# gudovskiy/contextflow

Hardware: AMD Instinct MI355X
Metric: samples/s fwd+logdet (log p(x) (B,M)), CIFAR-10C conv flow (higher is better)
Workload: dtype f32

## Files before the change

contextflow_amd/csrc/cf_step.hip:

```cpp
#include "cf_step_common.h"
#include <cstdlib>

namespace {

constexpr int kPrepBatch = 16;
struct StepPackBatch {
    const float *Wm[kPrepBatch], *t[kPrepBatch], *logs[kPrepBatch], *w1[kPrepBatch], *b1[kPrepBatch], *w2[kPrepBatch], *b2[kPrepBatch],
        *w3[kPrepBatch], *b3[kPrepBatch];
    float* ws[kPrepBatch];
    int pieces;
    int w24;
};
template <class G>
__global__ __launch_bounds__(256) void k_step_pack(const StepPackBatch pb) {
    const int bi = blockIdx.y;
    const float* __restrict__ Wm = pb.Wm[bi]; const float* __restrict__ t = pb.t[bi]; const float* __restrict__ logs = pb.logs[bi];
    const float* __restrict__ w1 = pb.w1[bi]; const float* __restrict__ b1 = pb.b1[bi]; const float* __restrict__ w2 = pb.w2[bi];
    const float* __restrict__ b2 = pb.b2[bi]; const float* __restrict__ w3 = pb.w3[bi]; const float* __restrict__ b3 = pb.b3[bi];
    float* __restrict__ ws = pb.ws[bi];
    const int gtid = blockIdx.x * 256 + threadIdx.x, gsz = gridDim.x * 256;
    if (gtid == 0) {
        float s = 0.f;
        for (int c = 0; c < G::C; ++c) s += logs[c];
        ws[0] = (float)G::HW * ws[1] + s;
// ... 34 lines not shown
    }
    {
        constexpr int HID = G::HID;
        const double Gm[4][3] = {{1, 0, 0}, {.5, .5, .5}, {.5, -.5, .5}, {0, 0, 1}};
        for (int e = gtid; e < 16 * HID * HID; e += gsz) {
            const int jj = e & 3, ln = (e >> 2) & 63, q = e >> 8;
            const int kg = q % G::KG4, rt16 = (q / G::KG4) % G::RT16, pos = q / (G::KG4 * G::RT16);
            const int co = rt16 * 16 + (ln & 15), ci = 4 * (4 * kg + jj) + (ln >> 4), xi = pos >> 2, nu = pos & 3;
            const float* wk = w2 + ((int64_t)co * HID + ci) * 9;
            double u = 0.0;
            for (int a = 0; a < 3; ++a)
                for (int b = 0; b < 3; ++b) u += Gm[xi][a] * Gm[nu][b] * (double)wk[a * 3 + b];
            ws[G::OFF_AW + e] = (float)u;
        }
        if (G::KB32 > 0 && G::HID == 32 && pb.pieces) {
            unsigned short* wb = reinterpret_cast<unsigned short*>(ws + G::OFF_AWB);
            for (int e = gtid; e < 16 * G::RT16 * G::KB32 * 64 * 8; e += gsz) {
                const int j = e & 7, ln = (e >> 3) & 63, q = e >> 9;
                const int kb = q % G::KB32, rt16 = (q / G::KB32) % G::RT16, pos = q / (G::KB32 * G::RT16);
                const int co = rt16 * 16 + (ln & 15), ci = 32 * kb + 4 * j + (ln >> 4), xi = pos >> 2, nu = pos & 3;
                const float* wk = w2 + ((int64_t)co * HID + ci) * 9;
                double u = 0.0;
                for (int a = 0; a < 3; ++a)
                    for (int b = 0; b < 3; ++b) u += Gm[xi][a] * Gm[nu][b] * (double)wk[a * 3 + b];
                const float uf = (float)u;
                const unsigned u0 = __float_as_uint(uf) & 0xffff0000u;
                const float r1 = uf - __uint_as_float(u0);
                const unsigned u1 = __float_as_uint(r1) & 0xffff0000u;
                const float r2 = r1 - __uint_as_float(u1);
                const unsigned pc[3] = {u0, u1, __float_as_uint(r2)};
#pragma unroll
                for (int pz = 0; pz < 3; ++pz)
                    wb[((((int64_t)(pos * G::RT16 + rt16) * G::KB32 + kb) * 3 + pz) * 64 + ln) * 8 + j] = (unsigned short)(pc[pz] >> 16);
            }
        }
        if (G::KB32 > 0 && G::HID == 32 && pb.pieces) {
            unsigned short* wb = reinterpret_cast<unsigned short*>(ws + G::OFF_ADB);
            for (int e = gtid; e < 9 * G::RT16 * G::KB32 * 64 * 8; e += gsz) {
                const int j = e & 7, ln = (e >> 3) & 63, q = e >> 9;
                const int kb = q % G::KB32, rt16 = (q / G::KB32) % G::RT16, tap = q / (G::KB32 * G::RT16);
                const int co = rt16 * 16 + (ln & 15), ci = 32 * kb + 8 * (ln >> 4) + j;
                const float uf = w2[((int64_t)co * HID + ci) * 9 + tap];
                const unsigned u0 = __float_as_uint(uf) & 0xffff0000u;
                const float r1 = uf - __uint_as_float(u0);
                const unsigned u1 = __float_as_uint(r1) & 0xffff0000u;
                const float r2 = r1 - __uint_as_float(u1);
                const unsigned pc[3] = {u0, u1, __float_as_uint(r2)};
#pragma unroll
                for (int pz = 0; pz < 3; ++pz)
                    wb[((((int64_t)(tap * G::RT16 + rt16) * G::KB32 + kb) * 3 + pz) * 64 + ln) * 8 + j] = (unsigned short)(pc[pz] >> 16);
            }
        }
    }
    if (G::H == 4 && G::W == 4 && pb.w24) {
        constexpr int HID = G::HID;
        const double G2[4][3] = {{1, 0, 0}, {.5, .5, .5}, {.5, -.5, .5}, {0, 0, 1}};
        const double G4[6][3] = {{4, 0, 0}, {2. / 3, 2. / 3, 2. / 3}, {2. / 3, -2. / 3, 2. / 3}, {-8. / 3, -4. / 3, -2. / 3},
                                 {-8. / 3, 4. / 3, -2. / 3}, {0, 0, 1}};
        for (int e = gtid; e < 24 * HID * HID; e += gsz) {
            const int jj = e & 3, ln = (e >> 2) & 63, q = e >> 8;
            const int kg = q % G::KG4, rt16 = (q / G::KG4) % G::RT16, pos = q / (G::KG4 * G::RT16);
            const int co = rt16 * 16 + (ln & 15), ci = 4 * (4 * kg + jj) + (ln >> 4), xi = pos / 6, nu = pos % 6;
            const float* wk = w2 + ((int64_t)co * HID + ci) * 9;
            double u = 0.0;
            for (int a = 0; a < 3; ++a)
                for (int b = 0; b < 3; ++b) u += G2[xi][a] * G4[nu][b] * (double)wk[a * 3 + b];
            ws[G::OFF_AW24 + e] = (float)u;
        }
    }
    if constexpr (G::RS16) {
        constexpr int C = G::C, HID = G::HID, HALF = G::HALF;
        for (int p = gtid; p < C; p += gsz) { ws[G::OFF_RB0 + p] = -t[p] * expf(-logs[p]); ws[G::OFF_RB3 + p] = b3[p]; }
        for (int p = gtid; p < HID; p += gsz) { ws[G::OFF_RB1 + p] = b1[p]; ws[G::OFF_RB2 + p] = b2[p]; }
        auto split16 = [](int e, int NG, int& rt, int& gi, int& row, int& kk, int& j) {
            j = e & 3; const int ln = (e >> 2) & 63, q = e >> 8; gi = q % NG; rt = q / NG; row = 16 * rt + (ln & 15); kk = ln >> 4;
        };
        int rt, gi, row, kk, j;
        for (int e = gtid; e < (C / 16) * (C / 16) * 256; e += gsz) {
            split16(e, C / 16, rt, gi, row, kk, j);
            const int k = 4 * (4 * gi + j) + kk;
            ws[G::OFF_RA0 + e] = expf(-logs[row]) * Wm[row * C + k];
        }
        for (int e = gtid; e < (HID / 16) * (HALF / 16) * 256; e += gsz) {
            split16(e, HALF / 16, rt, gi, row, kk, j);
            ws[G::OFF_RA1 + e] = w1[row * HALF + 4 * (4 * gi + j) + kk];
        }
        for (int e = gtid; e < (HID / 16) * 9 * (HID / 16) * 256; e += gsz) {
            split16(e, 9 * (HID / 16), rt, gi, row, kk, j);
            const int tap = gi / (HID / 16), ci = 4 * (4 * (gi % (HID / 16)) + j) + kk;
            ws[G::OFF_RA2 + e] = w2[(row * HID + ci) * 9 + tap];
        }
        for (int e = gtid; e < (C / 16) * (HID / 16) * 256; e += gsz) {
            split16(e, HID / 16, rt, gi, row, kk, j);
            ws[G::OFF_RA3 + e] = w3[row * HID + 4 * (4 * gi + j) + kk];
        }
    }
    if constexpr (G::SMALL) {
        for (int p = gtid; p < 16; p += gsz) {
            const int ch = chan_of_row16<G>(p);
            ws[G::OFF_SB0 + p] = ch >= 0 ? -t[ch] * expf(-logs[ch]) : 0.f;
            ws[G::OFF_SB3 + p] = ch >= 0 ? b3[ch] : 0.f;
        }
        for (int e = gtid; e < G::SG0 * 256; e += gsz) {
            const int jj = e & 3, ln = (e >> 2) & 63, gg = e >> 8, ch = chan_of_row16<G>(ln & 15), k = 4 * (4 * gg + jj) + (ln >> 4);
            ws[G::OFF_SA0 + e] = (ch >= 0 && k < G::C) ? expf(-logs[ch]) * Wm[ch * G::C + k] : 0.f;
        }
        for (int e = gtid; e < G::SG3 * 256; e += gsz) {
// ... 992 lines not shown
    float* Xp = H1 + C * PIX;
#pragma unroll
    for (int rt = 0; rt < I::RTI; ++rt)
#pragma unroll
        for (int q = 0; q < PTW; ++q)
#pragma unroll
            for (int r = 0; r < 16; ++r) {
                const int row = rt * 32 + tile_row(r, lk);
                if (row < C) Xp[row * PIX + pix[q]] = acc[rt][q][r];
            }
    cf_wave_sync();
    if (x_unsq) rows_store_unsq<G>(x, Xp, b0, B, wave, lane);
    else rows_store<G, C>(x, Xp, b0, 0, B, wave, lane);
}

template <class G>
int launch_prepare_inv(const float* Wm, const float* t, const float* logs, float* wsi, hipStream_t s) {
    using I = GeoInv<G>;
    int rc = cf_slogdet_inverse(Wm, G::C, wsi + I::WS_FLOATS, wsi + I::OFF_WINV, (cf_stream_t)s);
    if (rc) return rc;
    k_step_pack_inv<G><<<dim3(16), dim3(256), 0, s>>>(t, logs, wsi);
    return 0;
}

static int g_bf16_split = -1;
static int bf16_split_mode() {
    static const int v = [] { const char* e = getenv("CONTEXTFLOW_BF16_SPLIT"); return (e && (e[0] == '1' || e[0] == '2')) ? e[0] - '0' : 0; }();
    return g_bf16_split < 0 ? v : g_bf16_split;
}
static bool bf16_split_enabled() { return bf16_split_mode() != 0; }

template <class G>
int launch_step_inv(const float* z, float* x, const float* ws, const float* wsi, int B, int64_t zbs, int x_unsq, hipStream_t s) {
    constexpr size_t lds_bytes = (size_t)G::LDS_FLOATS * sizeof(float);
    if (lds_bytes > 64 * 1024) {
        static std::atomic<uint64_t> raised{0};
        if (int rc_ = cf_raise_dynamic_lds((const void*)k_flow_step_inv<G>, 160 * 1024, raised, __func__)) return rc_;
    }
    k_flow_step_inv<G><<<dim3((B + G::SPW - 1) / G::SPW), dim3(256), lds_bytes, s>>>(z, x, ws, wsi, B, zbs, x_unsq);
    return 0;
}


}

static bool direct_conv_only() {
    static const bool v = [] { const char* e = getenv("CONTEXTFLOW_DIRECT_CONV"); return e && e[0] == '1'; }();
    return v;
}
static bool wino24_enabled() {
    static const bool v = [] { const char* e = getenv("CONTEXTFLOW_WINO24"); return !(e && e[0] == '0'); }();
    return v;
}

extern "C" {

int cf_flow_step_supported(int C, int H, int W, int kh, int kw) {
    return (kh == 3 && kw == 3 && shape_id(C, H, W) >= 0) ? 1 : 0;
}

int64_t cf_flow_step_ws_bytes(int C, int H, int W) {
    switch (shape_id(C, H, W)) {
        case 0: return (int64_t)G8::WS_FLOATS * 4;
        case 1: return (int64_t)G16::WS_FLOATS * 4;
        case 2: return (int64_t)G32::WS_FLOATS * 4;
        case 3: return (int64_t)G64::WS_FLOATS * 4;
    }
    return 0;
}

int cf_flow_step_prepare_batch(int n, const float* const* Wm, const float* const* t, const float* const* logs, const float* const* w1,
                               const float* const* b1, const float* const* w2, const float* const* b2, const float* const* w3,
                               const float* const* b3, void* const* ws, float* const* winv, int C, int H, int W, cf_stream_t stream) {
    CF_REQUIRE(n >= 0 && Wm && t && logs && w1 && b1 && w2 && b2 && w3 && b3 && ws);
    const int sid = shape_id(C, H, W);
    if (sid < 0) { cf_set_error("cf_flow_step_prepare: shape (%d,%d,%d) unsupported", C, H, W); return CF_ERR_UNSUPPORTED; }
    for (int i0 = 0; i0 < n; i0 += kPrepBatch) {
        const int m = n - i0 < kPrepBatch ? n - i0 : kPrepBatch;
        StepPackBatch pb{};
        pb.pieces = bf16_split_enabled() ? 1 : 0;
        pb.w24 = (wino24_enabled() && !direct_conv_only()) ? 1 : 0;
        for (int i = 0; i < m; ++i) {
            const int j = i0 + i;
            CF_REQUIRE(Wm[j] && t[j] && logs[j] && w1[j] && b1[j] && w2[j] && b2[j] && w3[j] && b3[j] && ws[j] &&
                       (reinterpret_cast<uintptr_t>(ws[j]) & 15) == 0 && (!winv || winv[j]));
            pb.Wm[i] = Wm[j]; pb.t[i] = t[j]; pb.logs[i] = logs[j]; pb.w1[i] = w1[j]; pb.b1[i] = b1[j]; pb.w2[i] = w2[j]; pb.b2[i] = b2[j];
            pb.w3[i] = w3[j]; pb.b3[i] = b3[j]; pb.ws[i] = (float*)ws[j];
        }
        int rc = 0;
        switch (sid) {
            case 0: rc = launch_prepare<G8>(pb, m, winv ? winv + i0 : nullptr, cf_s(stream)); break;
            case 1: rc = launch_prepare<G16>(pb, m, winv ? winv + i0 : nullptr, cf_s(stream)); break;
            case 2: rc = launch_prepare<G32>(pb, m, winv ? winv + i0 : nullptr, cf_s(stream)); break;
            default: rc = launch_prepare<G64>(pb, m, winv ? winv + i0 : nullptr, cf_s(stream)); break;
        }
        if (rc) return rc;
        CF_LAUNCH_CHECK();
    }
    return 0;
}

int cf_flow_step_prepare(const float* Wm, const float* t, const float* logs, const float* w1, const float* b1,
                         const float* w2, const float* b2, const float* w3, const float* b3, void* ws, int C, int H, int W,
                         cf_stream_t stream) {
    CF_REQUIRE(Wm && t && logs && w1 && b1 && w2 && b2 && w3 && b3 && ws && (reinterpret_cast<uintptr_t>(ws) & 15) == 0);
    return cf_flow_step_prepare_batch(1, &Wm, &t, &logs, &w1, &b1, &w2, &b2, &w3, &b3, &ws, nullptr, C, H, W, stream);
// ... 71 lines not shown
    if (dbg != nullptr && variant == 3 && shape_id(C, H, W) <= 1 && shape_id(C, H, W) >= 0) {
        if (shape_id(C, H, W) == 0)
            rc = in_squeeze ? launch_step_small<G8s, true, true>(x, z, ldj_acc, w, B, x_bstride, cf_s(stream), dbg)
                            : launch_step_small<G8s, false, true>(x, z, ldj_acc, w, B, x_bstride, cf_s(stream), dbg);
        else
            rc = in_squeeze ? launch_step_small<G16s, true, true>(x, z, ldj_acc, w, B, x_bstride, cf_s(stream), dbg)
                            : launch_step_small<G16s, false, true>(x, z, ldj_acc, w, B, x_bstride, cf_s(stream), dbg);
        if (rc) return rc;
        CF_LAUNCH_CHECK();
        return 0;
    }
    if (dbg != nullptr) {
        CF_REQUIRE(variant == 0);
#define CF_STEPD(G) rc = in_squeeze ? launch_step<G, true, 0, false, true>(x, z, ldj_acc, w, B, x_bstride, dbg, flags, cf_s(stream)) \
                                    : launch_step<G, false, 0, false, true>(x, z, ldj_acc, w, B, x_bstride, dbg, flags, cf_s(stream))
        switch (shape_id(C, H, W)) {
            case 0: CF_STEPD(G8); break;
            case 1: CF_STEPD(G16); break;
            case 2: CF_STEPD(G32); break;
            case 3: CF_STEPD(G64); break;
            default: cf_set_error("cf_flow_step_fwd_debug: shape (%d,%d,%d) unsupported", C, H, W); return CF_ERR_UNSUPPORTED;
        }
#undef CF_STEPD
        if (rc) return rc;
        CF_LAUNCH_CHECK();
        return 0;
    }
    switch (shape_id(C, H, W) * 8 + variant) {
        case 0: CF_STEP(G8); break;
        case 3: rc = in_squeeze ? launch_step_small<G8s, true>(x, z, ldj_acc, w, B, x_bstride, cf_s(stream))
                                : launch_step_small<G8s, false>(x, z, ldj_acc, w, B, x_bstride, cf_s(stream)); break;
        case 8: CF_STEP(G16); break;
        case 9: CF_STEP(G16v1); break;
        case 10: CF_STEP(G16v2); break;
        case 11: rc = in_squeeze ? launch_step_small<G16s, true>(x, z, ldj_acc, w, B, x_bstride, cf_s(stream))
                                : launch_step_small<G16s, false>(x, z, ldj_acc, w, B, x_bstride, cf_s(stream)); break;
        case 16: CF_STEP(G32); break;
        case 17: CF_STEP(G32v1); break;
        case 18: CF_STEP(G32v2); break;
        case 19: CF_STEP(G32v3); break;
        case 24: CF_STEP(G64); break;
        case 25: CF_STEP(G64v1); break;
        case 26: CF_STEP(G64v2); break;
        case 27: CF_STEP(G64v3); break;
        case 4: rc = in_squeeze ? launch_step_small<G8w, true>(x, z, ldj_acc, w, B, x_bstride, cf_s(stream))
                               : launch_step_small<G8w, false>(x, z, ldj_acc, w, B, x_bstride, cf_s(stream)); break;
        case 14: rc = in_squeeze ? launch_step_small<G16wb, true>(x, z, ldj_acc, w, B, x_bstride, cf_s(stream))
                                 : launch_step_small<G16wb, false>(x, z, ldj_acc, w, B, x_bstride, cf_s(stream)); break;
        case 15: rc = in_squeeze ? launch_step_small<G16db, true>(x, z, ldj_acc, w, B, x_bstride, cf_s(stream))
                                 : launch_step_small<G16db, false>(x, z, ldj_acc, w, B, x_bstride, cf_s(stream)); break;
        case 12: rc = in_squeeze ? launch_step_small<G16w, true>(x, z, ldj_acc, w, B, x_bstride, cf_s(stream))
                                : launch_step_small<G16w, false>(x, z, ldj_acc, w, B, x_bstride, cf_s(stream)); break;
        case 20: CF_STEP(G32w); break;
        case 28: CF_STEP(G64w); break;
        case 29: CF_STEP(G64w2); break;
        case 30: CF_STEP(G64w24); break;
        default: cf_set_error("cf_flow_step_fwd: shape (%d,%d,%d) variant %d unsupported", C, H, W, variant); return CF_ERR_UNSUPPORTED;
    }
#undef CF_STEP
    if (rc) return rc;
    CF_LAUNCH_CHECK();
    return 0;
}

int cf_flow_step_chain_max_batch(int C, int H, int W) {
    switch (shape_id(C, H, W)) {
        case 0: case 1: return direct_conv_only() ? 0 : 1024;
        case 2: return 512;
        case 3: return CF_RS16_MAXB < CF_RS_MAXB_C64 ? CF_RS16_MAXB : CF_RS_MAXB_C64;
    }
    return 0;
}

int cf_flow_step_fwd_chain(const float* x, float* z, float* ldj_acc, const void* const* ws, int n, int B, int C, int H, int W,
                           int64_t x_bstride, int in_squeeze, cf_stream_t stream) {
    if (B == 0 || n == 0) return 0;
    CF_REQUIRE(x && z && ldj_acc && ws && n >= 1 && n <= kChain && B > 0 && x_bstride >= (int64_t)C * H * W);
    CF_REQUIRE((reinterpret_cast<uintptr_t>(x) & 15) == 0 && (reinterpret_cast<uintptr_t>(z) & 15) == 0 && x_bstride % 4 == 0);
    const int sid = shape_id(C, H, W);
    if (sid < 0 || B > cf_flow_step_chain_max_batch(C, H, W)) {
        cf_set_error("cf_flow_step_fwd_chain: shape (%d,%d,%d) at a batch of %d is not a chained case", C, H, W, B);
        return CF_ERR_UNSUPPORTED;
    }
    WsChain wc{};
    for (int i = 0; i < n; ++i) { CF_REQUIRE(ws[i]); wc.ws[i] = (const float*)ws[i]; }
    hipStream_t s = cf_s(stream);
    switch (sid) {
        case 0: in_squeeze ? launch_step_small_chain<G8w, true>(x, z, ldj_acc, wc, n, B, x_bstride, s)
                           : launch_step_small_chain<G8w, false>(x, z, ldj_acc, wc, n, B, x_bstride, s); break;
        case 1: in_squeeze ? launch_step_small_chain<G16w, true>(x, z, ldj_acc, wc, n, B, x_bstride, s)
                           : launch_step_small_chain<G16w, false>(x, z, ldj_acc, wc, n, B, x_bstride, s); break;
        case 2: in_squeeze ? launch_step_rs_chain<G32, 2, true>(x, z, ldj_acc, wc, n, B, x_bstride, s)
                           : launch_step_rs_chain<G32, 2, false>(x, z, ldj_acc, wc, n, B, x_bstride, s); break;
        default:
            if (in_squeeze) k_flow_step_rs16_chain<G64, true><<<dim3(B), dim3(256), 0, s>>>(x, z, ldj_acc, wc, n, B, x_bstride);
            else k_flow_step_rs16_chain<G64, false><<<dim3(B), dim3(256), 0, s>>>(x, z, ldj_acc, wc, n, B, x_bstride);
    }
    CF_LAUNCH_CHECK();
    return 0;
}

int cf_bf16_split(int on) {
    if (on >= 0) g_bf16_split = on > 2 ? 1 : on;
    return bf16_split_mode();
}

int cf_flow_step_fwd(const float* x, float* z, float* ldj_acc, const void* ws, int B, int C, int H, int W,
                     int64_t x_bstride, int in_squeeze, cf_stream_t stream) {
    int flags = 0;
    const int sid = shape_id(C, H, W);
    if ((sid == 2 && B < 256 * G32::SPW) || (sid == 3 && B < 256 * G64::SPW)) flags = 2 << 16;
    if (sid == 0 || sid == 1) flags = 3 << 16;
    const bool direct_only = direct_conv_only();
    if (!direct_only && (sid == 0 || sid == 1 || (sid == 2 && B >= 256 * G32::SPW))) flags = 4 << 16;
    if (!direct_only && sid == 3 && B >= 256 * G64w2::SPW) flags = (wino24_enabled() ? 6 : 5) << 16;
    if (!direct_only && sid == 1 && bf16_split_mode() == 1) flags = 6 << 16;
    if (!direct_only && sid == 1 && bf16_split_mode() == 2 && B >= 1024) flags = 7 << 16;
    if ((sid == 2 && B <= 512) || (sid == 3 && B <= CF_RS_MAXB_C64)) {
        CF_REQUIRE(x && z && ldj_acc && ws && B >= 0 && x_bstride >= (int64_t)C * H * W);
        if (B == 0) return 0;
        const float* w = (const float*)ws;
        if (sid == 3 && B <= CF_RS16_MAXB) {
            if (in_squeeze) k_flow_step_rs16<G64, true><<<dim3(B), dim3(256), 0, cf_s(stream)>>>(x, z, ldj_acc, w, B, x_bstride, kNoTape);
            else k_flow_step_rs16<G64, false><<<dim3(B), dim3(256), 0, cf_s(stream)>>>(x, z, ldj_acc, w, B, x_bstride, kNoTape);
            CF_LAUNCH_CHECK();
            return 0;
        }
        if (sid == 2) { if (in_squeeze) launch_step_rs<G32, 2, true>(x, z, ldj_acc, w, B, x_bstride, cf_s(stream));
                        else launch_step_rs<G32, 2, false>(x, z, ldj_acc, w, B, x_bstride, cf_s(stream)); }
        else          { if (in_squeeze) launch_step_rs<G64, 1, true>(x, z, ldj_acc, w, B, x_bstride, cf_s(stream));
                        else launch_step_rs<G64, 1, false>(x, z, ldj_acc, w, B, x_bstride, cf_s(stream)); }
        CF_LAUNCH_CHECK();
        return 0;
    }
    return cf_flow_step_fwd_debug(x, z, ldj_acc, ws, B, C, H, W, x_bstride, in_squeeze, nullptr, flags, stream);
}

int64_t cf_flow_step_macs(int B, int C, int H, int W, int pass) {
    const int sid = shape_id(C, H, W);
    if (sid < 0 || pass < 0 || pass > 3) return 0;
    const int64_t direct = 40ll * C * C * H * W, wino = 20ll * C * C * H * W, wino24 = 16ll * C * C * H * W;
    if (pass == 2 || direct_conv_only()) return direct;
    if (pass == 3) return wino;
    if (sid == 3 && pass == 0 && wino24_enabled() && B >= 256 * G64w2::SPW) return wino24;
    bool w;
    if (sid == 0) w = pass == 0;
    else if (sid == 1) w = true;
    else if (sid == 2) w = B >= 256 * G32::SPW;
    else w = B >= 256 * G64w2::SPW;
    return w ? wino : direct;
}

int64_t cf_flow_step_tape_aux_bytes(int B, int C, int H, int W) {
    return shape_id(C, H, W) < 0 ? 0 : tape_aux_bytes(B, C, H, W);
}

int cf_flow_step_fwd_taped(const float* x, float* z, float* ldj_acc, const void* ws, float* t_y0, float* t_h1, float* t_h2,
                           void* t_aux, int B, int C, int H, int W, int64_t x_bstride, int in_squeeze, cf_stream_t stream) {
    if (B == 0) return 0;
    CF_REQUIRE(x && z && ldj_acc && ws && t_y0 && t_h1 && t_h2 && t_aux && x_bstride >= (int64_t)C * H * W && x_bstride % 4 == 0);
    CF_REQUIRE((reinterpret_cast<uintptr_t>(x) & 15) == 0 && (reinterpret_cast<uintptr_t>(z) & 15) == 0 &&
               (reinterpret_cast<uintptr_t>(t_y0) & 15) == 0 && (reinterpret_cast<uintptr_t>(t_h1) & 15) == 0 &&
               (reinterpret_cast<uintptr_t>(t_h2) & 15) == 0 && (reinterpret_cast<uintptr_t>(t_aux) & 15) == 0);
    const float* w = (const float*)ws;
    const StepTape tp = make_tape(t_y0, t_h1, t_h2, t_aux, B, C, H, W);
    const bool direct_only = direct_conv_only();
    int rc = 0;
#define CF_STEPT(G) rc = in_squeeze ? launch_step<G, true, 0, true>(x, z, ldj_acc, w, B, x_bstride, nullptr, 0, cf_s(stream), nullptr, tp) \
                                    : launch_step<G, false, 0, true>(x, z, ldj_acc, w, B, x_bstride, nullptr, 0, cf_s(stream), nullptr, tp)
    switch (shape_id(C, H, W)) {
        case 0: rc = in_squeeze ? launch_step_small<G8s, true, false, true>(x, z, ldj_acc, w, B, x_bstride, cf_s(stream), nullptr, tp)
                                : launch_step_small<G8s, false, false, true>(x, z, ldj_acc, w, B, x_bstride, cf_s(stream), nullptr, tp); break;
        case 1: if (direct_only) rc = in_squeeze ? launch_step_small<G16s, true, false, true>(x, z, ldj_acc, w, B, x_bstride, cf_s(stream), nullptr, tp)
                                                 : launch_step_small<G16s, false, false, true>(x, z, ldj_acc, w, B, x_bstride, cf_s(stream), nullptr, tp);
                else rc = in_squeeze ? launch_step_small<G16w, true, false, true>(x, z, ldj_acc, w, B, x_bstride, cf_s(stream), nullptr, tp)
                                     : launch_step_small<G16w, false, false, true>(x, z, ldj_acc, w, B, x_bstride, cf_s(stream), nullptr, tp);
                break;
        case 2: if (B <= 512) rc = in_squeeze ? launch_step_rs<G32, 2, true, true>(x, z, ldj_acc, w, B, x_bstride, cf_s(stream), tp)
                                              : launch_step_rs<G32, 2, false, true>(x, z, ldj_acc, w, B, x_bstride, cf_s(stream), tp);
                else if (B < 256 * G32::SPW) CF_STEPT(G32v2); else if (direct_only) CF_STEPT(G32); else CF_STEPT(G32w); break;
        case 3: if (B <= CF_RS16_MAXB) {
                    if (in_squeeze) k_flow_step_rs16<G64, true, true><<<dim3(B), dim3(256), 0, cf_s(stream)>>>(x, z, ldj_acc, w, B, x_bstride, tp);
                    else k_flow_step_rs16<G64, false, true><<<dim3(B), dim3(256), 0, cf_s(stream)>>>(x, z, ldj_acc, w, B, x_bstride, tp);
                }
                else if (!direct_only && B >= 256 * G64w2::SPW) CF_STEPT(G64w2); else if (B < 256 * G64::SPW) CF_STEPT(G64v2); else CF_STEPT(G64); break;
        default: cf_set_error("cf_flow_step_fwd_taped: shape (%d,%d,%d) unsupported", C, H, W); return CF_ERR_UNSUPPORTED;
    }
#undef CF_STEPT
    if (rc) return rc;
    CF_LAUNCH_CHECK();
    return 0;
}

int cf_flow_step_fwd_ctx(const float* x, float* z, float* ldj_acc, const void* ws, const float* sbias, int mode, int B, int C,
                         int H, int W, int64_t x_bstride, cf_stream_t stream) {
    if (B == 0) return 0;
    const bool keep_direct = (mode & 4) != 0;
// ... 51 lines not shown
```

contextflow_amd/csrc/cf_step_common.h:

```cpp
#pragma once
#include <type_traits>
#include "cf_common.h"
#include <math.h>

namespace {


typedef float f32x16 __attribute__((ext_vector_type(16)));

constexpr int kWaves = 4;

template <int C_, int H_, int W_, int SPW_, int PIPE_ = 1, int ABL_ = 0, int PATCH_ = 0>
struct Geo {
    static constexpr int C = C_, H = H_, W = W_, SPW = SPW_, PIPE = PIPE_, ABL = ABL_, PATCH = PATCH_;
    static constexpr int HW = H * W;
    static constexpr int PIX = SPW * HW;
    static constexpr int HALF = C / 2;
    static constexpr int HID = 2 * C;
    static constexpr int NPT = PIX / 32;
    static constexpr int PTW = NPT / kWaves;
    static constexpr int HP = HALF <= 16 ? 16 : 32;
    static constexpr int R03 = 2 * HP;
    static constexpr int RT03 = R03 / 32;
    static constexpr int RT1 = (HID + 31) / 32;
    static constexpr int R1 = RT1 * 32;
    static constexpr int KS0 = C / 2, KS1 = HALF / 2, KS3 = HID / 2;
    static constexpr int NG0 = (KS0 + 3) / 4, NG1 = (KS1 + 3) / 4, NG3 = (KS3 + 3) / 4;
    static constexpr int NCG = HID / 8;
    static constexpr int NG2 = 9 * NCG;
    static constexpr int OFF_B0 = 4, OFF_B1 = OFF_B0 + R03, OFF_B2 = OFF_B1 + R1, OFF_B3 = OFF_B2 + R1;
    static constexpr int OFF_A0 = OFF_B3 + R03;
    static constexpr int OFF_A1 = OFF_A0 + NG0 * RT03 * 256;
    static constexpr int OFF_A2 = OFF_A1 + NG1 * RT1 * 256;
    static constexpr int OFF_A3 = OFF_A2 + NG2 * RT1 * 256;
    static constexpr bool SMALL = (H == 16 && W == 16 && SPW == 1 && C <= 16);
    static constexpr bool HID16 = SMALL && HID == 16;
    static constexpr int SG0 = (C + 15) / 16, SG3 = (HID + 15) / 16, SG1 = (HALF + 15) / 16;
    static constexpr int OFF_SB0 = OFF_A3 + NG3 * RT03 * 256;
    static constexpr int OFF_SB3 = OFF_SB0 + (SMALL ? 16 : 0);
    static constexpr int OFF_SA0 = OFF_SB3 + (SMALL ? 16 : 0);
    static constexpr int OFF_SA3 = OFF_SA0 + (SMALL ? SG0 * 256 : 0);
    static constexpr int OFF_SA1 = OFF_SA3 + (SMALL ? SG3 * 256 : 0);
    static constexpr int OFF_SA2 = OFF_SA1 + (HID16 ? SG1 * 256 : 0);
    static constexpr bool W24 = (PIPE_ == 6);
    static constexpr bool WINO = (PIPE_ == 3 || PIPE_ == 4 || W24);
    static constexpr bool BF16S = (PIPE_ == 4);
    static constexpr bool DBF = (PIPE_ == 5);
    static constexpr int RT16 = HID / 16, KG4 = HID / 16;
    static constexpr int OFF_AW = OFF_SA2 + (HID16 ? 9 * 256 : 0);
    static constexpr bool RS16 = (C == 64 && H == 4 && W == 4);
    static constexpr int OFF_RB0 = OFF_AW + 16 * HID * HID, OFF_RB1 = OFF_RB0 + C, OFF_RB2 = OFF_RB1 + HID, OFF_RB3 = OFF_RB2 + HID;
    static constexpr int OFF_RA0 = OFF_RB3 + C, OFF_RA1 = OFF_RA0 + (C / 16) * (C / 16) * 256;
    static constexpr int OFF_RA2 = OFF_RA1 + (HID / 16) * (HALF / 16) * 256, OFF_RA3 = OFF_RA2 + (HID / 16) * 9 * (HID / 16) * 256;
    static constexpr int R16_END = OFF_RA3 + (C / 16) * (HID / 16) * 256;
    static constexpr int WS_END0 = RS16 ? R16_END : OFF_AW + 16 * HID * HID;
    static constexpr int KB32 = HID / 32;
    static constexpr int OFF_AWB = WS_END0;
    static constexpr int OFF_ADB = WS_END0 + 16 * RT16 * KB32 * 3 * 256;
    static constexpr int OFF_AW24 = OFF_ADB + 9 * RT16 * KB32 * 3 * 256;
    static constexpr int WS_FLOATS = OFF_AW24 + ((H == 4 && W == 4) ? 24 * HID * HID : 0);
    static constexpr int PP = 2 * W + 2 * H + 4;
    static constexpr int RS = PATCH ? ((PIX + SPW * PP + 1 + 3) & ~3) : PIX;
#ifndef CF_WINO_LDSW
#define CF_WINO_LDSW 1
#endif
    static constexpr int LDS_W = (CF_WINO_LDSW && PIPE_ == 3 && HID == 16 && H == 16 && W == 16 && SPW == 1) ? 16 * HID * HID : 0;
    static constexpr int DBF_FLOATS = 3 * PIX * HID / 2;
    static constexpr int LDS_FLOATS = (DBF && DBF_FLOATS > (HALF + HID) * RS) ? DBF_FLOATS : (HALF + HID) * RS + LDS_W;
    static constexpr int MINW = (160 * 1024) / (LDS_FLOATS * 4) >= 4 ? 4 : ((160 * 1024) / (LDS_FLOATS * 4) >= 2 ? 2 : 1);
    static_assert(PIX % 128 == 0 && PTW >= 1, "workgroup must own a multiple of 128 pixels");
    static_assert(!W24 || (H == 4 && W == 4 && SPW == 8), "F(2x4, 3x3): 4x4 images, 8 samples = one column tile of 16 output tiles");
    static_assert(HID % 8 == 0 && C % 4 == 0, "channel counts must fill whole k-steps");
    static_assert((HW & (HW - 1)) == 0 && (W & (W - 1)) == 0, "power-of-two images");
};

template <class G> __host__ __device__ constexpr int chan_of_row(int p) {
    return ((p % G::HP) < G::HALF) ? (p / G::HP) * G::HALF + (p % G::HP) : -1;
}

template <class G> __host__ __device__ constexpr int chan_of_row16(int p) {
    return (2 * (p >> 2) + (p & 1) < G::HALF) ? ((p & 2) ? G::HALF : 0) + 2 * (p >> 2) + (p & 1) : -1;
}

__device__ __forceinline__ f32x16 bias_tile(const float* __restrict__ bias32, int lk) {
    f32x16 a;
#pragma unroll
    for (int q = 0; q < 4; ++q) {
        const float4 v = *reinterpret_cast<const float4*>(bias32 + 8 * q + 4 * lk);
        a[4 * q + 0] = v.x; a[4 * q + 1] = v.y; a[4 * q + 2] = v.z; a[4 * q + 3] = v.w;
    }
    return a;
}
__device__ __forceinline__ int tile_row(int r, int lk) { return (r & 3) + 8 * (r >> 2) + 4 * lk; }
__device__ __forceinline__ float cf_relu(float x) { return __int_as_float(max(__float_as_int(x), 0)); }
__device__ __forceinline__ float cf_log_scale(float raw) { return fmaf(-4.0f, __builtin_amdgcn_rcpf(__expf(raw) + 1.0f), 2.0f); }
__device__ __forceinline__ float f4e(const float4& v, int e) { return e == 0 ? v.x : e == 1 ? v.y : e == 2 ? v.z : v.w; }

template <int RT, int PTW>
struct GroupOps {
    float4 a[RT];
    float b[4][PTW];
};

template <int RT, int PTW>
__device__ __forceinline__ void group_mma(f32x16 (&acc)[RT][PTW], const GroupOps<RT, PTW>& o, int nsteps) {
#pragma unroll
    for (int e = 0; e < 4; ++e) {
        if (e < nsteps) {
#pragma unroll
            for (int q = 0; q < PTW; ++q)
#pragma unroll
                for (int rt = 0; rt < RT; ++rt)
                    acc[rt][q] = __builtin_amdgcn_mfma_f32_32x32x2f32(f4e(o.a[rt], e), o.b[e][q], acc[rt][q], 0, 0, 0);
        }
    }
}

typedef __amdgpu_buffer_rsrc_t ws_rsrc_t;
__device__ __forceinline__ ws_rsrc_t ws_rsrc(const float* ws, int floats) {
    return __builtin_amdgcn_make_buffer_rsrc(const_cast<float*>(ws), 0, floats * 4, 0x00020000);
}
__device__ __forceinline__ float4 ws_frag(ws_rsrc_t rs, int lane, int foff) {
    typedef int i32x4_t __attribute__((ext_vector_type(4)));
    const i32x4_t v = __builtin_amdgcn_raw_buffer_load_b128(rs, lane * 16, foff * 4, 0);
// ... 570 lines not shown
#pragma unroll
                for (int j = 0; j < 2; ++j)
                    if (AT[j][nu] != 0.f) {
                        const float k0 = c0 * AT[j][nu], k1 = c1 * AT[j][nu];
#pragma unroll
                        for (int ct = 0; ct < NT; ++ct)
#pragma unroll
                            for (int rt = 0; rt < RTW; ++rt) {
                                if constexpr (decltype(has0)::value) Y[ct][0][j][rt] += k0 * M[ct][rt];
                                if constexpr (decltype(has1)::value) Y[ct][1][j][rt] += k1 * M[ct][rt];
                            }
                    }
                __builtin_amdgcn_sched_barrier(0);
            }
#pragma unroll
            for (int ct = 0; ct < NT; ++ct) { r1[ct] = r1n[ct]; r2[ct] = r2n[ct]; }
        };
        if constexpr (CF_WINO_PEEL == 2) {
            xi_body(0, std::true_type{}, std::false_type{});
            xi_body(1, std::true_type{}, std::true_type{});
            xi_body(2, std::true_type{}, std::true_type{});
            xi_body(3, std::false_type{}, std::true_type{});
        } else if constexpr (CF_WINO_PEEL) {
            xi_body(0, std::true_type{}, std::false_type{});
#pragma unroll 1
            for (int xi = 1; xi < 3; ++xi) xi_body(xi, std::true_type{}, std::true_type{});
            xi_body(3, std::false_type{}, std::true_type{});
        } else {
#pragma unroll 1
            for (int xi = 0; xi < 4; ++xi) xi_body(xi, std::true_type{}, std::true_type{});
        }
    }
    }
    __syncthreads();
#pragma unroll
    for (int rt = 0; rt < RTW; ++rt) {
        const float4 b = *reinterpret_cast<const float4*>(wsl + G::OFF_B2 + (rt0 + rt) * 16 + 4 * lg);
#pragma unroll
        for (int ct = 0; ct < NT; ++ct)
#pragma unroll
            for (int i = 0; i < 2; ++i) {
                float* dst = H1 + ((rt0 + rt) * 16 + 4 * lg) * PIX + smp[ct] * HW + (2 * ty[ct] + i) * W + 2 * tx[ct];
                const float bb[4] = {b.x, b.y, b.z, b.w};
#pragma unroll
                for (int r = 0; r < 4; ++r)
                    *reinterpret_cast<float2*>(dst + r * PIX) =
                        make_float2(cf_relu(Y[ct][i][0][rt][r] + bb[r]), cf_relu(Y[ct][i][1][rt][r] + bb[r]));
            }
    }
    if constexpr (RSPLIT > 1) __syncthreads();
    else cf_wave_sync();
}

template <class G> __device__ __forceinline__ int w24_pix(int s, int y, int x, int kpar) { return 8 * (4 * y + ((x + y + kpar) & 3)) + s; }

template <class G>
__device__ __forceinline__ void winograd24_phase2(float* __restrict__ lds, const float* __restrict__ wsl, ws_rsrc_t rs, int lane,
                                                  int wave) {
    constexpr int W = G::W, H = G::H, HW = G::HW, PIX = G::PIX, HALF = G::HALF, RT16 = G::RT16, KG4 = G::KG4;
    static_assert(G::W24 && RT16 % 4 == 0, "F(2x4, 3x3) geometry");
    constexpr int RTW = RT16 / 4;
    constexpr int NS = 6 * KG4;
    constexpr int NU[6] = {0, 5, 1, 2, 3, 4};
    typedef float f32x2w __attribute__((ext_vector_type(2)));
    const int rt0 = __builtin_amdgcn_readfirstlane(wave * RTW);
    float* H1 = lds + HALF * PIX;
    const int l15 = lane & 15, lg = lane >> 4;
    const int smp = l15 >> 1, ty = l15 & 1;
    int yrow[4];
#pragma unroll
    for (int a = 0; a < 4; ++a) {
        const int yy = 2 * ty - 1 + a;
        yrow[a] = yy < 0 ? -yy : (yy >= H ? 2 * (H - 1) - yy : yy);
    }
    f32x4w Y[2][4][RTW];
#pragma unroll
    for (int i = 0; i < 2; ++i)
#pragma unroll
        for (int j = 0; j < 4; ++j)
#pragma unroll
            for (int rt = 0; rt < RTW; ++rt) Y[i][j][rt] = f32x4w{0.f, 0.f, 0.f, 0.f};
    auto addrs = [&](int xi, int (&o)[2][6]) {
#pragma unroll
        for (int h = 0; h < 2; ++h) {
            const int yy = h == 0 ? (xi == 0 ? yrow[0] : (xi == 2 ? yrow[2] : yrow[1]))
                                  : (xi == 2 ? yrow[1] : (xi == 3 ? yrow[3] : yrow[2]));
#pragma unroll
            for (int c = 0; c < 6; ++c) {
                const int xx = c == 0 ? 1 : (c == 5 ? 2 : c - 1);
                o[h][c] = 4 * (HALF * PIX + lg * PIX + w24_pix<G>(smp, yy, xx, lg & 1));
            }
        }
    };
    struct Raw { f32x2w d[2][6][2]; };
    struct WFrag { float4 a[RTW]; };
    auto load_raw = [&](const int (&o)[2][6], int kk, Raw& r) {
#pragma unroll
        for (int h = 0; h < 2; ++h)
#pragma unroll
            for (int c = 0; c < 6; ++c)
#pragma unroll
                for (int e2 = 0; e2 < 2; ++e2) {
                    const char* q0 = reinterpret_cast<const char*>(lds) + (16 * kk + 8 * e2) * PIX * 4;
                    const char* q1 = q0 + 4 * PIX * 4;
                    r.d[h][c][e2] = f32x2w{*reinterpret_cast<const float*>(q0 + o[h][c]), *reinterpret_cast<const float*>(q1 + o[h][c])};
                }
    };
    auto load_w = [&](int xi, int s, WFrag& f) {
        const int kk = s / 6, nu = NU[s % 6];
        const int fr = G::OFF_AW24 + (((xi * 6 + nu) * RT16 + rt0) * KG4 + kk) * 256;
#pragma unroll
        for (int rt = 0; rt < RTW; ++rt) f.a[rt] = ws_frag(rs, lane, fr + rt * KG4 * 256);
    };
    int o[2][6];
    addrs(0, o);
    Raw raw;
    WFrag wf[2];
    load_raw(o, 0, raw);
    load_w(0, 0, wf[0]);
    auto xi_body = [&](const int xi, auto has0, auto has1) {
        const int xn = xi < 3 ? xi + 1 : 3;
        const float sigma = xi == 1 ? 1.f : -1.f;
        const float c0 = xi < 3 ? 1.f : 0.f, c1 = xi == 0 ? 0.f : (xi == 1 ? 1.f : -1.f);
        f32x4w M[6][RTW];
#pragma unroll
        for (int nu = 0; nu < 6; ++nu)
#pragma unroll
            for (int rt = 0; rt < RTW; ++rt) M[nu][rt] = f32x4w{0.f, 0.f, 0.f, 0.f};
#pragma unroll
        for (int kk = 0; kk < KG4; ++kk) {
            f32x2w A[6][2];
#pragma unroll
            for (int c = 0; c < 6; ++c)
#pragma unroll
                for (int e2 = 0; e2 < 2; ++e2) A[c][e2] = raw.d[0][c][e2] + sigma * raw.d[1][c][e2];
            if (kk + 1 < KG4) {
                load_raw(o, kk + 1, raw);
            } else {
                addrs(xn, o);
                load_raw(o, 0, raw);
            }
#pragma unroll
            for (int t = 0; t < 6; ++t) {
                const int s = kk * 6 + t, nu = NU[t];
                if (s + 1 < NS) load_w(xi, s + 1, wf[(s + 1) & 1]);
                else load_w(xn, 0, wf[0]);
                __builtin_amdgcn_sched_barrier(0);
                f32x2w v[2];
#pragma unroll
                for (int e2 = 0; e2 < 2; ++e2) {
                    const f32x2w a0 = A[0][e2], a1 = A[1][e2], a2 = A[2][e2], a3 = A[3][e2], a4 = A[4][e2], a5 = A[5][e2];
                    if (nu == 0) v[e2] = 0.25f * a0 + (a4 - 1.25f * a2);
                    else if (nu == 1) v[e2] = (a4 - 0.25f * a2) + (a3 - 0.25f * a1);
                    else if (nu == 2) v[e2] = (a4 - 0.25f * a2) - (a3 - 0.25f * a1);
                    else if (nu == 3) v[e2] = (a4 - a2) + 0.5f * (a3 - a1);
                    else if (nu == 4) v[e2] = (a4 - a2) - 0.5f * (a3 - a1);
                    else v[e2] = 0.25f * a1 + (a5 - 1.25f * a3);
                }
                const WFrag& f = wf[s & 1];
#pragma unroll
                for (int e = 0; e < 4; ++e)
#pragma unroll
                    for (int rt = 0; rt < RTW; ++rt)
                        M[nu][rt] = __builtin_amdgcn_mfma_f32_16x16x4f32(f4e(f.a[rt], e), v[e >> 1][e & 1], M[nu][rt], 0, 0, 0);
                __builtin_amdgcn_sched_barrier(0);
            }
        }
#pragma unroll
        for (int rt = 0; rt < RTW; ++rt) {
            const f32x4w s12 = M[1][rt] + M[2][rt], d12 = M[1][rt] - M[2][rt], s34 = M[3][rt] + M[4][rt], d34 = M[3][rt] - M[4][rt];
            const f32x4w Z[4] = {M[0][rt] + s12 + s34, d12 + 0.5f * d34, s12 + 0.25f * s34, d12 + 0.125f * d34 + M[5][rt]};
#pragma unroll
            for (int j = 0; j < 4; ++j) {
                if constexpr (decltype(has0)::value) Y[0][j][rt] += c0 * Z[j];
                if constexpr (decltype(has1)::value) Y[1][j][rt] += c1 * Z[j];
            }
        }
    };
    xi_body(0, std::true_type{}, std::false_type{});
#pragma unroll 1
    for (int xi = 1; xi < 3; ++xi) xi_body(xi, std::true_type{}, std::true_type{});
    xi_body(3, std::false_type{}, std::true_type{});
    __syncthreads();
#pragma unroll
    for (int rt = 0; rt < RTW; ++rt) {
        const float4 b = *reinterpret_cast<const float4*>(wsl + G::OFF_B2 + (rt0 + rt) * 16 + 4 * lg);
        const float bb[4] = {b.x, b.y, b.z, b.w};
#pragma unroll
        for (int i = 0; i < 2; ++i)
#pragma unroll
            for (int r = 0; r < 4; ++r) {
                float* dst = H1 + ((rt0 + rt) * 16 + 4 * lg + r) * PIX + smp * HW + (2 * ty + i) * W;
                *reinterpret_cast<float4*>(dst) = make_float4(cf_relu(Y[i][0][rt][r] + bb[r]), cf_relu(Y[i][1][rt][r] + bb[r]),
                                                              cf_relu(Y[i][2][rt][r] + bb[r]), cf_relu(Y[i][3][rt][r] + bb[r]));
            }
    }
    __syncthreads();
}

template <class G>
__device__ __forceinline__ void direct_bf16_phases(float* __restrict__ lds, const float* __restrict__ wsl, ws_rsrc_t rs, int lane, int wave) {
    static_assert(G::DBF && G::H == 16 && G::W == 16 && G::SPW == 1 && G::HID == 32 && G::PTW == 2, "the 16x16 level at C = 16");
    constexpr int PIX = G::PIX, HALF = G::HALF, HID = G::HID, PTW = G::PTW, RT16 = G::RT16;
    constexpr int PLANE = PIX * HID * 2;
    typedef __bf16 bf16x8w __attribute__((ext_vector_type(8)));
    float* Y0 = lds;
    float* H1 = lds + HALF * PIX;
    char* const ldsb = reinterpret_cast<char*>(lds);
    const int li = lane & 31, lk = lane >> 5, l15 = lane & 15, lg = lane >> 4;
    int pix[PTW];
#pragma unroll
    for (int q = 0; q < PTW; ++q) pix[q] = (wave * PTW + q) * 32 + li;
    f32x16 acc1[1][PTW];
#pragma unroll
    for (int q = 0; q < PTW; ++q) acc1[0][q] = bias_tile(wsl + G::OFF_B1, lk);
    dense_phase<G, G::KS1, G::NG1, 1>(acc1, rs, G::OFF_A1, Y0, pix, lane);
    float4 wp[2][RT16][3];
    auto wp_load = [&](float4 (&dst)[RT16][3], int tap) {
#pragma unroll
        for (int rt = 0; rt < RT16; ++rt)
#pragma unroll
            for (int pz = 0; pz < 3; ++pz) dst[rt][pz] = ws_frag(rs, lane, G::OFF_ADB + ((tap * RT16 + rt) * 3 + pz) * 256);
    };
    wp_load(wp[0], 0);
    __syncthreads();
#pragma unroll
    for (int q = 0; q < PTW; ++q) {
        const int xx = pix[q] & 15;
#pragma unroll
        for (int a = 0; a < 4; ++a) {
            unsigned p[3][4];
#pragma unroll
            for (int i = 0; i < 4; ++i) {
                const float v = cf_relu(acc1[0][q][4 * a + i]);
#ifdef CF_ABL_DB_NOSPLIT
                p[0][i] = p[1][i] = p[2][i] = __float_as_uint(v);
                continue;
#endif
                const unsigned u0 = __float_as_uint(v) & 0xffff0000u;
                const float r1 = v - __uint_as_float(u0);
                const unsigned u1 = __float_as_uint(r1) & 0xffff0000u;
                const float r2 = r1 - __uint_as_float(u1);
                p[0][i] = u0; p[1][i] = u1; p[2][i] = __float_as_uint(r2);
            }
            char* dst = ldsb + pix[q] * (HID * 2) + ((a ^ ((xx >> 1) & 2)) * 16) + lk * 8;
// ... 50 lines not shown
    }
    __syncthreads();
#pragma unroll
    for (int rt = 0; rt < RT16; ++rt) {
        const float4 bv = *reinterpret_cast<const float4*>(wsl + G::OFF_B2 + rt * 16 + 4 * lg);
        const float bb[4] = {bv.x, bv.y, bv.z, bv.w};
#pragma unroll
        for (int ct = 0; ct < 4; ++ct)
#pragma unroll
            for (int r = 0; r < 4; ++r) H1[(rt * 16 + 4 * lg + r) * PIX + wave * 64 + 16 * ct + l15] = cf_relu(acc[ct][rt][r] + bb[r]);
    }
    cf_wave_sync();
}

template <class G, int CTX = 0, bool DUMP = false, int UPTO = 3>
__device__ __forceinline__ void conditioner_net(f32x16 (&acc3)[G::RT03][G::PTW], float* __restrict__ lds,
                                                const float* __restrict__ wsl, const int (&pix)[G::PTW],
                                                const int (&pin)[G::PTW], int lane, int tid, float* __restrict__ dbg,
                                                int64_t dbg_cols, int tile, const float* __restrict__ sb = nullptr,
                                                const int* soff = nullptr, StepTape tp = kNoTape, int B = 0) {
    constexpr int C = G::C, W = G::W, H = G::H, PIX = G::PIX, HALF = G::HALF, HID = G::HID;
    constexpr int PTW = G::PTW, RT03 = G::RT03, RT1 = G::RT1;
    float* Y0 = lds;
    float* H1 = lds + HALF * PIX;
    const int lk = lane >> 5;
    const ws_rsrc_t rs = ws_rsrc(wsl, G::WS_FLOATS);
    {
        f32x16 acc[RT1][PTW];
#pragma unroll
        for (int rt = 0; rt < RT1; ++rt)
#pragma unroll
            for (int q = 0; q < PTW; ++q) acc[rt][q] = bias_tile(wsl + G::OFF_B1 + rt * 32, lk);
        if constexpr (CTX == 2) {
#pragma unroll
            for (int rt = 0; rt < RT1; ++rt)
#pragma unroll
                for (int q = 0; q < PTW; ++q)
#pragma unroll
                    for (int r = 0; r < 16; ++r) {
                        const int row = rt * 32 + tile_row(r, lk);
                        if (row < HID) acc[rt][q][r] += sb[soff[q] + row];
                    }
        }
        dense_phase<G, G::KS1, G::NG1, RT1>(acc, rs, G::OFF_A1, Y0, pix, lane);
        if constexpr (G::WINO && (G::HW > 32 * PTW || G::W24)) __syncthreads();
#pragma unroll
        for (int rt = 0; rt < RT1; ++rt)
#pragma unroll
            for (int q = 0; q < PTW; ++q)
#pragma unroll
                for (int r = 0; r < 16; ++r) {
                    const int row = rt * 32 + tile_row(r, lk);
                    if constexpr (G::W24) {
                        const int pw = w24_pix<G>((pix[q] - pin[q]) / G::HW, pin[q] / W, pin[q] % W, r & 1);
                        if (row < HID) H1[row * PIX + pw] = cf_relu(acc[rt][q][r]);
                    } else if constexpr (G::WINO) {
                        const int pw = wino_pix<G>(pix[q] - pin[q], pin[q] / W, pin[q] % W) ^ ((r & 1) * (W / 2));
                        if (row < HID) H1[row * PIX + pw] = cf_relu(acc[rt][q][r]);
                    } else {
                        if (row < HID) H1[row * PIX + pix[q]] = cf_relu(acc[rt][q][r]);
                    }
                }
        if constexpr (DUMP && G::WINO) {
#pragma unroll
            for (int q = 0; q < PTW; ++q) {
                const int b = tile * G::SPW + (pix[q] - pin[q]) / G::HW;
                if (b < B) {
                    float* dst = tp.h1 + (int64_t)b * HID * G::HW + pin[q];
#pragma unroll
                    for (int rt = 0; rt < RT1; ++rt)
#pragma unroll
                        for (int r = 0; r < 16; ++r) {
                            const int row = rt * 32 + tile_row(r, lk);
                            if (row < HID) dst[row * G::HW] = cf_relu(acc[rt][q][r]);
                        }
                }
            }
            mask_store<G, RT1>(tp.m1, acc, tile, tid >> 6, lane);
        } else if constexpr (DUMP) {
            cf_wave_sync();
            rows_store_t<G, HID, HID>(tp.h1, H1, tile * G::SPW, B, tid >> 6, lane);
            mask_store<G, RT1>(tp.m1, acc, tile, tid >> 6, lane);
        }
    }
    __syncthreads();
    if (dbg) {
        float* d = dbg + (int64_t)C * dbg_cols;
        for (int e = tid; e < HID * PIX; e += 256) d[(int64_t)(e / PIX) * dbg_cols + (int64_t)tile * PIX + (e % PIX)] = H1[e];
    }

    if constexpr (G::WINO) {
        if constexpr (G::W24) {
            static_assert(!DUMP, "the F(2x4) form runs in the evaluation forward only");
            winograd24_phase2<G>(lds, wsl, rs, lane, tid >> 6);
        } else {
            winograd_phase2<G>(lds, wsl, rs, lane, tid >> 6);
        }
        if constexpr (DUMP) {
            rows_store_t<G, HID, HID>(tp.h2, H1, tile * G::SPW, B, tid >> 6, lane);
#pragma unroll
            for (int rt = 0; rt < RT1; ++rt)
#pragma unroll
                for (int q = 0; q < PTW; ++q) {
                    unsigned bits = 0;
#pragma unroll
                    for (int r = 0; r < 16; ++r) {
                        const int row = rt * 32 + tile_row(r, lk);
// ... 143 lines not shown
            rows_store_t<G, HID, HID>(tp.h2, H1, tile * G::SPW, B, tid >> 6, lane);
            mask_store<G, RT1>(tp.m2, acc, tile, tid >> 6, lane);
        }
    }
    if (dbg) {
        __syncthreads();
        float* d = dbg + (int64_t)(C + HID) * dbg_cols;
        for (int e = tid; e < HID * PIX; e += 256) d[(int64_t)(e / PIX) * dbg_cols + (int64_t)tile * PIX + (e % PIX)] = H1[e];
    }

    if constexpr (UPTO < 3) return;
#pragma unroll
    for (int rt = 0; rt < RT03; ++rt)
#pragma unroll
        for (int q = 0; q < PTW; ++q) acc3[rt][q] = bias_tile(wsl + G::OFF_B3 + rt * 32, lk);
    if constexpr (CTX == 1) {
#pragma unroll
        for (int rt = 0; rt < RT03; ++rt)
#pragma unroll
            for (int q = 0; q < PTW; ++q)
#pragma unroll
                for (int r = 0; r < 16; ++r) {
                    const int ch = chan_of_row<G>(rt * 32 + (r & 3) + 8 * (r >> 2)) ;
                    const int ch1 = chan_of_row<G>(rt * 32 + (r & 3) + 8 * (r >> 2) + 4);
                    const int c = lk ? ch1 : ch;
                    if ((lk ? ch1 : ch) >= 0) acc3[rt][q][r] += sb[soff[q] + c];
                }
    }
    dense_phase<G, G::KS3, G::NG3, RT03>(acc3, rs, G::OFF_A3, H1, pix, lane);
}

using G8 = Geo<8, 16, 16, 1, 0>;
using G16 = Geo<16, 16, 16, 1, 0>;
using G32 = Geo<32, 8, 8, 4, 1>;
using G64 = Geo<64, 4, 4, 16, 1>;
using G16s = Geo<16, 16, 16, 1, 2>;
using G8s = Geo<8, 16, 16, 1, 2>;
using G16v1 = Geo<16, 16, 16, 1, 1>;
using G16v2 = Geo<16, 16, 16, 2, 1>;
using G32v1 = Geo<32, 8, 8, 4, 0>;
using G32v2 = Geo<32, 8, 8, 2, 1>;
using G32v3 = Geo<32, 8, 8, 8, 0>;
using G64v1 = Geo<64, 4, 4, 16, 1, 1>;
using G64v2 = Geo<64, 4, 4, 8, 1>;
using G64v3 = Geo<64, 4, 4, 16, 0>;
using G8w = Geo<8, 16, 16, 1, 3>;
using G16wb = Geo<16, 16, 16, 1, 4>;
using G16db = Geo<16, 16, 16, 1, 5>;
using G16w = Geo<16, 16, 16, 1, 3>;
using G32w = Geo<32, 8, 8, 4, 3>;
using G64w = Geo<64, 4, 4, 16, 3>;
using G64w2 = Geo<64, 4, 4, 8, 3>;
using G64w24 = Geo<64, 4, 4, 8, 6>;


int shape_id(int C, int H, int W) {
    if (C == 8 && H == 16 && W == 16) return 0;
    if (C == 16 && H == 16 && W == 16) return 1;
    if (C == 32 && H == 8 && W == 8) return 2;
    if (C == 64 && H == 4 && W == 4) return 3;
    return -1;
}

}
```

Before: 3.617 million.

## Extend F(2x4,3x3) Winograd hidden conv path to the 8x8 C=32 level

Generalizes the F(2x4, 3x3) Winograd second-conv phase, which previously only served the 4x4 C=64 level, so it also handles 8x8 images with 4 samples per workgroup spread over two column tiles. It adds a new LDS pixel swizzle for 8x8, per-lane tile x/y indexing, workspace sizing and weight-transform packing for the new geometry. It also enables this path by default for the 32x8x8 level at large batch, with an environment variable to turn it off. The aim is to cut the multiply count of the 3x3 hidden convolution at this level, at the cost of more transform work and a more complex LDS layout that may cause bank conflicts.

```diff
diff --git a/contextflow_amd/csrc/cf_step.hip b/contextflow_amd/csrc/cf_step.hip
--- a/contextflow_amd/csrc/cf_step.hip
+++ b/contextflow_amd/csrc/cf_step.hip
@@ -110,7 +110,7 @@
             }
         }
     }
-    if (G::H == 4 && G::W == 4 && pb.w24) {
+    if (G::HAS_W24 && pb.w24) {
         constexpr int HID = G::HID;
         const double G2[4][3] = {{1, 0, 0}, {.5, .5, .5}, {.5, -.5, .5}, {0, 0, 1}};
         const double G4[6][3] = {{4, 0, 0}, {2. / 3, 2. / 3, 2. / 3}, {2. / 3, -2. / 3, 2. / 3}, {-8. / 3, -4. / 3, -2. / 3},
@@ -1209,6 +1209,11 @@
     static const bool v = [] { const char* e = getenv("CONTEXTFLOW_WINO24"); return !(e && e[0] == '0'); }();
     return v;
 }
+static bool wino24_8x8_enabled() {
+    static const bool v = [] { const char* e = getenv("CONTEXTFLOW_WINO24_8X8"); return !(e && e[0] == '0'); }();
+    return v && wino24_enabled();
+}
+constexpr int kW24MinB8x8 = 512 * G32w24::SPW;
 
 extern "C" {
 
@@ -1386,6 +1391,7 @@
         case 12: rc = in_squeeze ? launch_step_small<G16w, true>(x, z, ldj_acc, w, B, x_bstride, cf_s(stream))
                                 : launch_step_small<G16w, false>(x, z, ldj_acc, w, B, x_bstride, cf_s(stream)); break;
         case 20: CF_STEP(G32w); break;
+        case 22: CF_STEP(G32w24); break;
         case 28: CF_STEP(G64w); break;
         case 29: CF_STEP(G64w2); break;
         case 30: CF_STEP(G64w24); break;
@@ -1448,6 +1454,7 @@
     const bool direct_only = direct_conv_only();
     if (!direct_only && (sid == 0 || sid == 1 || (sid == 2 && B >= 256 * G32::SPW))) flags = 4 << 16;
     if (!direct_only && sid == 3 && B >= 256 * G64w2::SPW) flags = (wino24_enabled() ? 6 : 5) << 16;
+    if (!direct_only && sid == 2 && B >= kW24MinB8x8 && wino24_8x8_enabled()) flags = 6 << 16;
     if (!direct_only && sid == 1 && bf16_split_mode() == 1) flags = 6 << 16;
     if (!direct_only && sid == 1 && bf16_split_mode() == 2 && B >= 1024) flags = 7 << 16;
     if ((sid == 2 && B <= 512) || (sid == 3 && B <= CF_RS_MAXB_C64)) {
@@ -1477,6 +1484,7 @@
     if (pass == 2 || direct_conv_only()) return direct;
     if (pass == 3) return wino;
     if (sid == 3 && pass == 0 && wino24_enabled() && B >= 256 * G64w2::SPW) return wino24;
+    if (sid == 2 && pass == 0 && wino24_8x8_enabled() && B >= kW24MinB8x8) return wino24;
     bool w;
     if (sid == 0) w = pass == 0;
     else if (sid == 1) w = true;
diff --git a/contextflow_amd/csrc/cf_step_common.h b/contextflow_amd/csrc/cf_step_common.h
--- a/contextflow_amd/csrc/cf_step_common.h
+++ b/contextflow_amd/csrc/cf_step_common.h
@@ -57,8 +57,9 @@
     static constexpr int KB32 = HID / 32;
     static constexpr int OFF_AWB = WS_END0;
     static constexpr int OFF_ADB = WS_END0 + 16 * RT16 * KB32 * 3 * 256;
+    static constexpr bool HAS_W24 = (H == 4 && W == 4) || (H == 8 && W == 8);
     static constexpr int OFF_AW24 = OFF_ADB + 9 * RT16 * KB32 * 3 * 256;
-    static constexpr int WS_FLOATS = OFF_AW24 + ((H == 4 && W == 4) ? 24 * HID * HID : 0);
+    static constexpr int WS_FLOATS = OFF_AW24 + (HAS_W24 ? 24 * HID * HID : 0);
     static constexpr int PP = 2 * W + 2 * H + 4;
     static constexpr int RS = PATCH ? ((PIX + SPW * PP + 1 + 3) & ~3) : PIX;
 #ifndef CF_WINO_LDSW
@@ -69,7 +70,8 @@
     static constexpr int LDS_FLOATS = (DBF && DBF_FLOATS > (HALF + HID) * RS) ? DBF_FLOATS : (HALF + HID) * RS + LDS_W;
     static constexpr int MINW = (160 * 1024) / (LDS_FLOATS * 4) >= 4 ? 4 : ((160 * 1024) / (LDS_FLOATS * 4) >= 2 ? 2 : 1);
     static_assert(PIX % 128 == 0 && PTW >= 1, "workgroup must own a multiple of 128 pixels");
-    static_assert(!W24 || (H == 4 && W == 4 && SPW == 8), "F(2x4, 3x3): 4x4 images, 8 samples = one column tile of 16 output tiles");
+    static_assert(!W24 || (H == 4 && W == 4 && SPW == 8) || (H == 8 && W == 8 && SPW == 4),
+                  "F(2x4, 3x3): 4x4 images, 8 samples = one column tile of 16 output tiles; 8x8 images, 4 samples = two column tiles");
     static_assert(HID % 8 == 0 && C % 4 == 0, "channel counts must fill whole k-steps");
     static_assert((HW & (HW - 1)) == 0 && (W & (W - 1)) == 0, "power-of-two images");
 };
@@ -746,27 +748,50 @@
     else cf_wave_sync();
 }
 
-template <class G> __device__ __forceinline__ int w24_pix(int s, int y, int x, int kpar) { return 8 * (4 * y + ((x + y + kpar) & 3)) + s; }
+template <class G> __device__ __forceinline__ int w24_row(int s, int y, int kq) {
+    return 128 * (s >> 1) + 32 * ((y ^ (kq >> 1)) & 1) + 8 * (y >> 1) + 4 * (s & 1);
+}
+template <class G> __device__ __forceinline__ int w24_col(int x, int kq) {
+    return 64 * ((x >> 1) & 1) + 2 * (((x >> 2) ^ (x >> 1)) & 1) + ((x ^ kq) & 1);
+}
+template <class G> __device__ __forceinline__ int w24_pix(int s, int y, int x, int kq) {
+    if constexpr (G::H == 4) return 8 * (4 * y + ((x + y + kq) & 3)) + s;
+    else return w24_row<G>(s, y, kq) + w24_col<G>(x, kq);
+}
 
 template <class G>
 __device__ __forceinline__ void winograd24_phase2(float* __restrict__ lds, const float* __restrict__ wsl, ws_rsrc_t rs, int lane,
                                                   int wave) {
     constexpr int W = G::W, H = G::H, HW = G::HW, PIX = G::PIX, HALF = G::HALF, RT16 = G::RT16, KG4 = G::KG4;
-    static_assert(G::W24 && RT16 % 4 == 0, "F(2x4, 3x3) geometry");
-    constexpr int RTW = RT16 / 4;
+    constexpr int NCT = PIX / 128;
+    constexpr int RSP = kWaves / NCT;
+    static_assert(G::W24 && (NCT == 1 || NCT == 2) && RT16 % RSP == 0 && W % 4 == 0, "F(2x4, 3x3) geometry");
+    constexpr int RTW = RT16 / RSP;
+    constexpr int TPS = HW / 8, TXN = W / 4;
     constexpr int NS = 6 * KG4;
     constexpr int NU[6] = {0, 5, 1, 2, 3, 4};
     typedef float f32x2w __attribute__((ext_vector_type(2)));
-    const int rt0 = __builtin_amdgcn_readfirstlane(wave * RTW);
+    const int rt0 = __builtin_amdgcn_readfirstlane((NCT == 1 ? wave : wave / NCT) * RTW);
     float* H1 = lds + HALF * PIX;
     const int l15 = lane & 15, lg = lane >> 4;
-    const int smp = l15 >> 1, ty = l15 & 1;
-    int yrow[4];
+    const int tg = (wave % NCT) * 16 + l15;
+    const int smp = H == 4 ? l15 >> 1 : tg / TPS, ty = H == 4 ? l15 & 1 : (tg % TPS) / TXN, tx = H == 4 ? 0 : tg % TXN;
+    int yrow[4], xcol[6];
 #pragma unroll
     for (int a = 0; a < 4; ++a) {
         const int yy = 2 * ty - 1 + a;
         yrow[a] = yy < 0 ? -yy : (yy >= H ? 2 * (H - 1) - yy : yy);
     }
+#pragma unroll
+    for (int c = 0; c < 6; ++c) {
+        const int xx = 4 * tx - 1 + c;
+        xcol[c] = xx < 0 ? -xx : (xx >= W ? 2 * (W - 1) - xx : xx);
+    }
+    int cpart[6];
+    if constexpr (H != 4) {
+#pragma unroll
+        for (int c = 0; c < 6; ++c) cpart[c] = 4 * (HALF * PIX + lg * PIX + w24_col<G>(xcol[c], lg));
+    }
     f32x4w Y[2][4][RTW];
 #pragma unroll
     for (int i = 0; i < 2; ++i)
@@ -781,8 +806,12 @@
                                   : (xi == 2 ? yrow[1] : (xi == 3 ? yrow[3] : yrow[2]));
 #pragma unroll
             for (int c = 0; c < 6; ++c) {
-                const int xx = c == 0 ? 1 : (c == 5 ? 2 : c - 1);
-                o[h][c] = 4 * (HALF * PIX + lg * PIX + w24_pix<G>(smp, yy, xx, lg & 1));
+                if constexpr (H == 4) {
+                    const int xx = c == 0 ? 1 : (c == 5 ? 2 : c - 1);
+                    o[h][c] = 4 * (HALF * PIX + lg * PIX + w24_pix<G>(smp, yy, xx, lg & 1));
+                } else {
+                    o[h][c] = 4 * w24_row<G>(smp, yy, lg) + cpart[c];
+                }
             }
         }
     };
@@ -884,7 +913,7 @@
         for (int i = 0; i < 2; ++i)
 #pragma unroll
             for (int r = 0; r < 4; ++r) {
-                float* dst = H1 + ((rt0 + rt) * 16 + 4 * lg + r) * PIX + smp * HW + (2 * ty + i) * W;
+                float* dst = H1 + ((rt0 + rt) * 16 + 4 * lg + r) * PIX + smp * HW + (2 * ty + i) * W + (H == 4 ? 0 : 4 * tx);
                 *reinterpret_cast<float4*>(dst) = make_float4(cf_relu(Y[i][0][rt][r] + bb[r]), cf_relu(Y[i][1][rt][r] + bb[r]),
                                                               cf_relu(Y[i][2][rt][r] + bb[r]), cf_relu(Y[i][3][rt][r] + bb[r]));
             }
@@ -1041,7 +1070,7 @@
                 for (int r = 0; r < 16; ++r) {
                     const int row = rt * 32 + tile_row(r, lk);
                     if constexpr (G::W24) {
-                        const int pw = w24_pix<G>((pix[q] - pin[q]) / G::HW, pin[q] / W, pin[q] % W, r & 1);
+                        const int pw = w24_pix<G>((pix[q] - pin[q]) / G::HW, pin[q] / W, pin[q] % W, G::H == 4 ? r & 1 : r & 3);
                         if (row < HID) H1[row * PIX + pw] = cf_relu(acc[rt][q][r]);
                     } else if constexpr (G::WINO) {
                         const int pw = wino_pix<G>(pix[q] - pin[q], pin[q] / W, pin[q] % W) ^ ((r & 1) * (W / 2));
@@ -1291,6 +1320,7 @@
 using G64w = Geo<64, 4, 4, 16, 3>;
 using G64w2 = Geo<64, 4, 4, 8, 3>;
 using G64w24 = Geo<64, 4, 4, 8, 6>;
+using G32w24 = Geo<32, 8, 8, 4, 6>;
 
 
 int shape_id(int C, int H, int W) {
```

Result: faster. 3.702 million, median of 6 (+2.4%).
